# eloialonso/diamond

Hardware: AMD Instinct MI355X
Metric: imagined frames/sec (64x64, 3 denoise steps, batch 256) (higher is better)
Workload: dtype f32 via split-f16 MFMA (world-model convs (3x3 stride 1 / 2, 1x1): fp32 operands split into 2 x fp16 pieces, 3 x v_mfma_f32_*_f16 per product, fp32 accumulate (fp32-class, 22-bit operands); attention core, linears: exact fp32 v_mfma_f32_16x16x4_f32; actor-critic encoder forward, dgrad and weight-gra

## Files before the change

diamond_amd/csrc/dmd_common.h:

```cpp
#pragma once
#include <atomic>
#include <hip/hip_runtime.h>
#include <stdint.h>
#include <stdio.h>
#include <stdlib.h>

#include "../../include/diamond_hip.h"

typedef float f32x4 __attribute__((ext_vector_type(4)));

#define DMD_GN_EPS 1e-5
#define DMD_MAX_DEVICES 16

#ifndef DMD_DYNAMIC_LDS
#define DMD_DYNAMIC_LDS(type, name) extern __shared__ __attribute__((aligned(16))) type name[]
#endif

void dmd_set_error(const char* fmt, ...);

int dmd_env_generation();
struct DmdEnvInt {
  const char* name;
  int def;
  std::atomic<long long> gen_val{-1};
// ... 2 lines not shown
    long long gv = gen_val.load(std::memory_order_acquire);
    if (gv < 0 || (int)(gv >> 32) != g) {
      const char* e = getenv(name);
      const int v = e ? atoi(e) : def;
      gv = ((long long)g << 32) | (unsigned int)v;
      gen_val.store(gv, std::memory_order_release);
    }
    return (int)(unsigned int)(gv & 0xffffffffll);
  }
};

#define DMD_CHECK_ARG(cond, ...)  \
  do {                            \
    if (!(cond)) {                \
      dmd_set_error(__VA_ARGS__); \
      return 1;                   \
    }                             \
  } while (0)

#define DMD_LAUNCH_CHECK()                                            \
  do {                                                                \
    hipError_t e_ = hipGetLastError();                                \
    if (e_ != hipSuccess) {                                           \
      dmd_set_error("launch failed: %s", hipGetErrorString(e_));      \
      return 2;                                                       \
    }                                                                 \
  } while (0)

__device__ __forceinline__ float dmd_silu(float v) { return v / (1.0f + expf(-v)); }
__device__ __forceinline__ float dmd_silu_fast(float t) {
  return t * __builtin_amdgcn_rcpf(1.0f + __builtin_amdgcn_exp2f(-1.4426950408889634f * t));
}
__device__ __forceinline__ float dmd_sigmoid(float v) { return 1.0f / (1.0f + expf(-v)); }

__device__ __forceinline__ void dmd_finalize_stats(const double* st, int T, double count, float* mean, float* rstd) {
  double s = 0.0, ss = 0.0;
  for (int t = 0; t < T; ++t) {
    s += st[2 * t];
    ss += st[2 * t + 1];
  }
  const double m = s / count;
  double var = ss / count - m * m;
  var = var < 0.0 ? 0.0 : var;
  *mean = (float)m;
  *rstd = (float)(1.0 / sqrt(var + (double)DMD_GN_EPS));
}

__device__ __forceinline__ double dmd_wave_sum(double v) {
#pragma unroll
  for (int off = 32; off > 0; off >>= 1) v += __shfl_xor(v, off, 64);
  return v;
}

__host__ __device__ __forceinline__ int dmd_gn_groups(int C) { return C / DMD_GN_GROUP > 0 ? C / DMD_GN_GROUP : 1; }
__host__ __device__ __forceinline__ int dmd_gn_group_size(int C) { return C / dmd_gn_groups(C); }
__host__ __device__ __forceinline__ bool dmd_gn_width_ok(int C) {
  return C > 0 && C % 16 == 0 && C % dmd_gn_groups(C) == 0 && dmd_gn_group_size(C) % 4 == 0 && (C % DMD_GN_GROUP == 0 || C <= 256);
}

__device__ __forceinline__ void norm_entry_gs(const dmd_norm& nm, int n, int c, int C, int gs, double count, float* mean,
                                              float* a, float* add) {
  const int G = C / gs;
  const int g = c / gs;
  float m, rstd;
  dmd_finalize_stats(nm.stats + ((size_t)(n * G + g) * nm.stat_tiles) * 2, nm.stat_tiles, count, &m, &rstd);
  float mul = nm.mul ? nm.mul[(size_t)n * nm.mul_stride + c] : 1.0f;
// ... 19 lines not shown
```

diamond_amd/csrc/dmd_linear.hip:

```cpp
#include "dmd_common.h"

#define LIN_DEPTH 4
template <bool SPLITK>
__global__ __launch_bounds__(256) void linear_mfma_kernel(const dmd_linear_params p) {
  __shared__ f32x4 part[SPLITK ? 3 : 1][4][64];
  const int lane = threadIdx.x & 63, wave = threadIdx.x >> 6;
  const int i = lane & 15, kg = lane >> 4;
  const int m0 = SPLITK ? blockIdx.x * 32 : blockIdx.x * 64 + (wave >> 1) * 32;
  const int n0 = SPLITK ? blockIdx.y * 32 : blockIdx.y * 64 + (wave & 1) * 32;
  const int kq = SPLITK ? p.K >> 2 : p.K;
  const int kbase = SPLITK ? wave * kq : 0;
  const int nsteps = kq >> 4;
  f32x4 acc[2][2];
#pragma unroll
  for (int a = 0; a < 2; ++a)
#pragma unroll
    for (int b = 0; b < 2; ++b) acc[a][b] = (f32x4){0.f, 0.f, 0.f, 0.f};

  const float* arow[2];
  const float* wrow[2];
#pragma unroll
  for (int b = 0; b < 2; ++b) {
    int m = m0 + 16 * b + i;
    m = m < p.M ? m : p.M - 1;
    arow[b] = p.A + (size_t)m * p.lda + kbase + 4 * kg;
    int n = n0 + 16 * b + i;
    n = n < p.N ? n : p.N - 1;
    wrow[b] = p.W + (size_t)n * p.ldw + kbase + 4 * kg;
  }
  f32x4 af[LIN_DEPTH][2], wf[LIN_DEPTH][2];
#pragma unroll
  for (int d = 0; d < LIN_DEPTH; ++d) {
    const int ks = (d < nsteps ? d : nsteps - 1) * 16;
#pragma unroll
    for (int b = 0; b < 2; ++b) {
      af[d][b] = *(const f32x4*)(arow[b] + ks);
      wf[d][b] = *(const f32x4*)(wrow[b] + ks);
    }
  }
  for (int s0 = 0; s0 < nsteps; s0 += LIN_DEPTH) {
#pragma unroll
    for (int d = 0; d < LIN_DEPTH; ++d) {
// ... 32 lines not shown
        for (int mb = 0; mb < 2; ++mb) acc[nb][mb] += part[w][nb * 2 + mb][lane];
  }
#pragma unroll
  for (int nb = 0; nb < 2; ++nb)
#pragma unroll
    for (int mb = 0; mb < 2; ++mb) {
      const int m = m0 + 16 * mb + i;
      const int n = n0 + 16 * nb + 4 * kg;
      if (m >= p.M) continue;
#pragma unroll
      for (int r = 0; r < 4; ++r) {
        if (n + r >= p.N) continue;
        float v = acc[nb][mb][r];
        if (p.bias) v += p.bias[n + r];
        float* c = p.C + (size_t)m * p.ldc + n + r;
        if (p.accumulate) v += *c;
        if (p.silu) v = dmd_silu(v);
        *c = v;
      }
    }
}

extern "C" int dmd_linear(const dmd_linear_params* p, dmd_stream_t stream) {
  DMD_CHECK_ARG(p && p->A && p->W && p->C, "linear: null");
  DMD_CHECK_ARG(p->M > 0 && p->N > 0 && p->K > 0 && p->K % 16 == 0, "linear: bad M/N/K %d %d %d", p->M, p->N, p->K);
  DMD_CHECK_ARG(p->lda % 4 == 0 && p->ldw % 4 == 0, "linear: lda/ldw must be multiples of 4");
  if (p->K >= 512 && p->K % 64 == 0)
    hipLaunchKernelGGL(linear_mfma_kernel<true>, dim3((p->M + 31) / 32, (p->N + 31) / 32), dim3(256), 0, (hipStream_t)stream, *p);
  else
    hipLaunchKernelGGL(linear_mfma_kernel<false>, dim3((p->M + 63) / 64, (p->N + 63) / 64), dim3(256), 0, (hipStream_t)stream, *p);
  DMD_LAUNCH_CHECK();
  return 0;
}
```

diamond_amd/csrc/dmd_pointwise.hip:

```cpp
#include "dmd_common.h"

__global__ void edm_pack_input_kernel(const float* __restrict__ x, const float* __restrict__ obs,
                                      const float* __restrict__ cond, int cond_stride, float sd,
                                      float* __restrict__ out, int N, int Cx, int Cobs, int HW, int CPad, int T, int head) {
  const int Q = CPad >> 2, HW4 = HW >> 2;
  const size_t idx = (size_t)blockIdx.x * blockDim.x + threadIdx.x;
  if (idx >= (size_t)N * HW4 * Q) return;
  const int qd = idx % Q;
  const size_t npq = idx / Q;
  const int n = npq / HW4;
  const int pix0 = 4 * (int)(npq - (size_t)n * HW4);
  const float c_in = cond[(size_t)n * cond_stride + 0];
  const int cimg = Cobs / T;
  f32x4 t[4];
#pragma unroll
  for (int e = 0; e < 4; ++e) {
    const int cc = qd * 4 + e;
    t[e] = (f32x4){0.f, 0.f, 0.f, 0.f};
    if (cc < Cobs) {
      const int fr = cc / cimg, ci = cc - fr * cimg;
      int slot = fr + head;
      slot = slot >= T ? slot - T : slot;
      const f32x4 v = *(const f32x4*)(obs + ((size_t)n * Cobs + slot * cimg + ci) * HW + pix0);
#pragma unroll
// ... 215 lines not shown
  const int ox = op % Wo;
  const int oy = (op / Wo) % Ho;
  const int n = op / ((size_t)Wo * Ho);
  f32x4 best;
  int bi[4] = {0, 0, 0, 0};
#pragma unroll
  for (int k = 0; k < 4; ++k) {
    const int iy = oy * 2 + (k >> 1), ix = ox * 2 + (k & 1);
    const f32x4 v = *(const f32x4*)(x + (((size_t)n * H + iy) * W + ix) * C + cq * 4);
    if (k == 0)
      best = v;
    else {
#pragma unroll
      for (int e = 0; e < 4; ++e)
        if (v[e] > best[e] || v[e] != v[e]) {
          best[e] = v[e];
          bi[e] = k;
        }
    }
  }
  *(f32x4*)(out + op * C + cq * 4) = best;
  if (argmax) {
    uint32_t packed = bi[0] | (bi[1] << 8) | (bi[2] << 16) | (bi[3] << 24);
    *(uint32_t*)(argmax + op * C + cq * 4) = packed;
  }
}

__global__ void lstm_pointwise_kernel(const float* __restrict__ gates, const float* __restrict__ c_prev,
                                      float* __restrict__ h, float* __restrict__ c, int N, int Hd) {
  const int idx = blockIdx.x * blockDim.x + threadIdx.x;
  if (idx >= N * Hd) return;
  const int n = idx / Hd, k = idx - n * Hd;
  const float* gr = gates + (size_t)n * 4 * Hd;
  const float ig = dmd_sigmoid(gr[k]);
  const float fg = dmd_sigmoid(gr[Hd + k]);
  const float gg = tanhf(gr[2 * Hd + k]);
  const float og = dmd_sigmoid(gr[3 * Hd + k]);
  const float cn = fg * c_prev[idx] + ig * gg;
  c[idx] = cn;
  h[idx] = og * tanhf(cn);
}

__global__ void lstm_pointwise_bwd_kernel(const float* __restrict__ gates, const float* __restrict__ c_prev,
                                          const float* __restrict__ c_new, const float* __restrict__ dh,
                                          const float* __restrict__ dc, float* __restrict__ dgates, float* __restrict__ dc_prev,
                                          int N, int Hd) {
  const int idx = blockIdx.x * blockDim.x + threadIdx.x;
  if (idx >= N * Hd) return;
  const int n = idx / Hd, k = idx - n * Hd;
  const float* gr = gates + (size_t)n * 4 * Hd;
  const float ig = dmd_sigmoid(gr[k]);
  const float fg = dmd_sigmoid(gr[Hd + k]);
  const float gg = tanhf(gr[2 * Hd + k]);
  const float og = dmd_sigmoid(gr[3 * Hd + k]);
  const float tc = tanhf(c_new[idx]);
  const float dhv = dh ? dh[idx] : 0.f;
  const float dcv = (dc ? dc[idx] : 0.f) + dhv * og * (1.0f - tc * tc);
  float* dg = dgates + (size_t)n * 4 * Hd;
  dg[k] = dcv * gg * ig * (1.0f - ig);
  dg[Hd + k] = dcv * c_prev[idx] * fg * (1.0f - fg);
  dg[2 * Hd + k] = dcv * ig * (1.0f - gg * gg);
  dg[3 * Hd + k] = dhv * tc * og * (1.0f - og);
  dc_prev[idx] = dcv * fg;
}

__global__ void categorical_sample_kernel(const float* __restrict__ logits, const float* __restrict__ expo,
                                          int64_t* __restrict__ out, int N, int A) {
  const int n = blockIdx.x * blockDim.x + threadIdx.x;
  if (n >= N) return;
  const float* l = logits + (size_t)n * A;
  const float* e = expo + (size_t)n * A;
  float m = -INFINITY;
  for (int a = 0; a < A; ++a) m = fmaxf(m, l[a]);
// ... 386 lines not shown
```

diamond_amd/lstm_native.py:

```python
from __future__ import annotations

from typing import Optional, Tuple

import torch
import torch.nn.functional as F
from torch import Tensor

from . import engine as E
from . import native as nv


def _pad_k(t: Tensor) -> Tensor:
    k = t.shape[1]
    kp = (k + 15) // 16 * 16
    t = t.contiguous()
    return t if kp == k else F.pad(t, (0, kp - k))


def _mm_nt(a: Tensor, w: Tensor, bias: Optional[Tensor] = None, out: Optional[Tensor] = None, accumulate: bool = False) -> Tensor:
    a, w = _pad_k(a), _pad_k(w)
    return E.linear(a, w, bias, out=out, accumulate=accumulate)


class LstmHeadsFn(torch.autograd.Function):
    @staticmethod
    def forward(ctx, cache: E.PackCache, x: Tensor, hx: Tensor, cx: Tensor, w_ih: Tensor, w_hh: Tensor, b_ih: Tensor,
                b_hh: Tensor, w_heads: Tensor, b_heads: Tensor):
        x, hx, cx = x.detach().float().contiguous(), hx.detach().float().contiguous(), cx.detach().float().contiguous()
        n, hd = hx.shape
        gates = E.linear(x, w_ih.detach(), b_ih.detach())
        E.linear(hx, w_hh.detach(), b_hh.detach(), out=gates, accumulate=True)
        h = torch.empty_like(hx)
        c = torch.empty_like(cx)
        nv.check(nv.lib().dmd_lstm_pointwise(nv.fptr(gates), nv.fptr(cx), nv.fptr(h), nv.fptr(c), n, hd, nv.stream()),
                 "dmd_lstm_pointwise")
        heads = E.linear(h, w_heads.detach().contiguous(), b_heads.detach().contiguous())
        ctx.save_for_backward(x, hx, cx, gates, h, c, w_heads)
        ctx.w_ih_t = cache.get(w_ih, "T", lambda w: w.detach().t().contiguous()) if ctx.needs_input_grad[1] else None
        ctx.w_hh_t = cache.get(w_hh, "T", lambda w: w.detach().t().contiguous()) if ctx.needs_input_grad[2] else None
        return heads, h, c

    @staticmethod
    def backward(ctx, dheads: Optional[Tensor], dh: Optional[Tensor], dc: Optional[Tensor]):
        x, hx, cx, gates, h, c, w_heads = ctx.saved_tensors
        n, hd = hx.shape
        need = ctx.needs_input_grad
        dw_heads = db_heads = None
        dh_total = None if dh is None else dh.detach().float().contiguous()
        if dheads is not None:
            dheads = dheads.detach().float().contiguous()
            wt = w_heads.detach().t().contiguous()
            dh_total = _mm_nt(dheads, wt, out=dh_total.clone() if dh_total is not None else None, accumulate=dh_total is not None)
            dw_heads = _mm_nt(dheads.t(), h.t())
            db_heads = dheads.sum(0)
        dgates = torch.empty_like(gates)
        dc_prev = torch.empty_like(cx)
        dcc = None if dc is None else dc.detach().float().contiguous()
        nv.check(nv.lib().dmd_lstm_pointwise_bwd(nv.fptr(gates), nv.fptr(cx), nv.fptr(c), nv.fptr(dh_total), nv.fptr(dcc),
                                                 nv.fptr(dgates), nv.fptr(dc_prev), n, hd, nv.stream()), "dmd_lstm_pointwise_bwd")
        dx = dhx = None
        if need[1]:
            dx = _mm_nt(dgates, ctx.w_ih_t)
        if need[2]:
            dhx = _mm_nt(dgates, ctx.w_hh_t)
        dgt = dgates.t().contiguous()
        dw_ih = _mm_nt(dgt, x.t())
        dw_hh = _mm_nt(dgt, hx.t())
        db = dgates.sum(0)
        return (None, dx, dhx, dc_prev if need[3] else None, dw_ih, dw_hh, db, db, dw_heads, db_heads)


class LinearFn(torch.autograd.Function):

    @staticmethod
    def forward(ctx, cache: E.PackCache, x: Tensor, w: Tensor, b: Optional[Tensor]):
        x = x.detach().float().contiguous()
        y = _mm_nt(x, w.detach(), None if b is None else b.detach().contiguous())
        ctx.save_for_backward(x)
        ctx.w_t = (cache.get(w, "T", lambda t: t.detach().t().contiguous()) if isinstance(w, torch.nn.Parameter)
                   else w.detach().t().contiguous()) if ctx.needs_input_grad[1] else None
        ctx.has_bias = b is not None
        return y

    @staticmethod
    def backward(ctx, dy: Tensor):
        (x,) = ctx.saved_tensors
        dy = dy.detach().float().contiguous()
        dx = _mm_nt(dy, ctx.w_t) if ctx.needs_input_grad[1] else None
        dw = _mm_nt(dy.t(), x.t())
        return None, dx, dw, dy.sum(0) if ctx.has_bias else None


class LstmStepFn(torch.autograd.Function):

    @staticmethod
    def forward(ctx, cache: E.PackCache, gx: Tensor, hx: Tensor, cx: Tensor, w_hh: Tensor, b_hh: Tensor):
        hx, cx = hx.detach().float().contiguous(), cx.detach().float().contiguous()
        n, hd = hx.shape
        gates = gx.detach().float().clone(memory_format=torch.contiguous_format)
        E.linear(hx, w_hh.detach(), b_hh.detach(), out=gates, accumulate=True)
        h, c = torch.empty_like(hx), torch.empty_like(cx)
        nv.check(nv.lib().dmd_lstm_pointwise(nv.fptr(gates), nv.fptr(cx), nv.fptr(h), nv.fptr(c), n, hd, nv.stream()),
                 "dmd_lstm_pointwise")
        ctx.save_for_backward(hx, cx, gates, c)
        ctx.w_hh_t = cache.get(w_hh, "T", lambda w: w.detach().t().contiguous())
        return h, c

    @staticmethod
    def backward(ctx, dh: Optional[Tensor], dc: Optional[Tensor]):
        hx, cx, gates, c = ctx.saved_tensors
        n, hd = hx.shape
        dhc = None if dh is None else dh.detach().float().contiguous()
        dcc = None if dc is None else dc.detach().float().contiguous()
        dgates, dc_prev = torch.empty_like(gates), torch.empty_like(cx)
        nv.check(nv.lib().dmd_lstm_pointwise_bwd(nv.fptr(gates), nv.fptr(cx), nv.fptr(c), nv.fptr(dhc), nv.fptr(dcc),
                                                 nv.fptr(dgates), nv.fptr(dc_prev), n, hd, nv.stream()), "dmd_lstm_pointwise_bwd")
        need = ctx.needs_input_grad
        dhx = _mm_nt(dgates, ctx.w_hh_t) if need[2] else None
        dw_hh = _mm_nt(dgates.t(), hx.t())
        return None, dgates, dhx, dc_prev if need[3] else None, dw_hh, dgates.sum(0)


class LstmBurnInFn(torch.autograd.Function):

    @staticmethod
    def forward(ctx, cache: E.PackCache, x: Tensor, tb: int, w_ih: Tensor, w_hh: Tensor, b_ih: Tensor, b_hh: Tensor):
        x = x.detach().float().contiguous()
        k, hd = x.shape[0] // tb, w_hh.shape[1]
        gates = E.linear(x, w_ih.detach(), b_ih.detach())
        hs = torch.zeros(tb + 1, k, hd, device=x.device, dtype=torch.float32)
        cs = torch.zeros(tb + 1, k, hd, device=x.device, dtype=torch.float32)
        whh, bhh = w_hh.detach(), b_hh.detach()
        for i in range(tb):
            g = gates[i * k:(i + 1) * k]
            E.linear(hs[i], whh, bhh, out=g, accumulate=True)
            nv.check(nv.lib().dmd_lstm_pointwise(nv.fptr(g), nv.fptr(cs[i]), nv.fptr(hs[i + 1]), nv.fptr(cs[i + 1]), k, hd, nv.stream()),
                     "dmd_lstm_pointwise")
        ctx.save_for_backward(x, gates, hs, cs)
        ctx.tb = tb
        ctx.w_ih_t = cache.get(w_ih, "T", lambda w: w.detach().t().contiguous()) if ctx.needs_input_grad[1] else None
        ctx.w_hh_t = cache.get(w_hh, "T", lambda w: w.detach().t().contiguous())
        return hs[tb].clone(), cs[tb].clone()

    @staticmethod
    def backward(ctx, dh: Optional[Tensor], dc: Optional[Tensor]):
        x, gates, hs, cs = ctx.saved_tensors
        tb = ctx.tb
        k, hd = hs.shape[1], hs.shape[2]
        dgates = torch.empty_like(gates)
        dhc = torch.zeros(k, hd, device=x.device) if dh is None else dh.detach().float().contiguous()
        dcc = torch.zeros(k, hd, device=x.device) if dc is None else dc.detach().float().contiguous()
        for i in reversed(range(tb)):
            dg, dc_prev = dgates[i * k:(i + 1) * k], torch.empty_like(dcc)
            nv.check(nv.lib().dmd_lstm_pointwise_bwd(nv.fptr(gates[i * k:(i + 1) * k]), nv.fptr(cs[i]), nv.fptr(cs[i + 1]), nv.fptr(dhc), nv.fptr(dcc),
                                                     nv.fptr(dg), nv.fptr(dc_prev), k, hd, nv.stream()), "dmd_lstm_pointwise_bwd")
            dcc = dc_prev
            if i > 0:
                dhc = _mm_nt(dg, ctx.w_hh_t)
        dx = _mm_nt(dgates, ctx.w_ih_t) if ctx.needs_input_grad[1] else None
        dgt = dgates.t().contiguous()
        dw_ih = _mm_nt(dgt, x.t())
        dw_hh = _mm_nt(dgt[:, k:].contiguous(), hs[1:tb].reshape((tb - 1) * k, hd).t()) if tb > 1 else torch.zeros_like(ctx.w_hh_t.t())
        db = dgates.sum(0)
        return None, dx, None, dw_ih, dw_hh, db, db


def lstm_burn_in(cache: E.PackCache, x: Tensor, tb: int, lstm) -> Tuple[Tensor, Tensor]:
    nv.require_gpu(x)
    return LstmBurnInFn.apply(cache, x, tb, lstm.weight_ih, lstm.weight_hh, lstm.bias_ih, lstm.bias_hh)

# ... 42 lines not shown
```

diamond_amd/native.py:

```python
from __future__ import annotations

import ctypes as C
import os
from typing import Optional

import torch
from torch import Tensor

_HERE = os.path.dirname(os.path.abspath(__file__))
LIB_PATH = os.environ.get("DIAMOND_LIB", os.path.join(_HERE, "libdiamond_hip.so"))

PROLOGUE_NONE, PROLOGUE_NORM_SILU, PROLOGUE_NORM = 0, 1, 2
PRECISION_F32, PRECISION_F16X2 = 0, 1
GN_GROUP = 32


class NativeLibraryMissing(RuntimeError):
    pass


class Norm(C.Structure):
    _fields_ = [("stats", C.c_void_p), ("stat_tiles", C.c_int32), ("mul_plus_one", C.c_int32), ("mul", C.c_void_p),
                ("add", C.c_void_p), ("mul_stride", C.c_int64), ("add_stride", C.c_int64)]

# ... 52 lines not shown

CHECKSUM_PARTS = 8


class PoolRound(C.Structure):
    _fields_ = [("frames", C.c_void_p), ("pad", C.c_void_p), ("act", C.c_void_p), ("hx", C.c_void_p), ("cx", C.c_void_p),
                ("is_f32", C.c_int32), ("rows", C.c_int32)]


class ResetSlotsParams(C.Structure):
    _fields_ = [("B", C.c_int32), ("K", C.c_int32), ("T", C.c_int32), ("head", C.c_int32), ("per_frame", C.c_int64),
                ("hd", C.c_int32), ("reserved", C.c_int32), ("pool", PoolRound * 2), ("pool_base", C.c_int64), ("num_dead", C.c_void_p),
                ("slot_row", C.c_void_p), ("row_slot", C.c_void_p), ("next_obs", C.c_void_p), ("ctx", C.c_void_p),
                ("act_ring", C.c_void_p), ("hx", C.c_void_p), ("cx", C.c_void_p), ("enc_in", C.c_void_p)]


CHAIN_MAX_BLOCKS = 8


class ChainBlock(C.Structure):
    _fields_ = [("skip_slot", C.c_int32), ("save_slot", C.c_int32), ("film1_mul", C.c_int32 * 2), ("film1_add", C.c_int32 * 2),
                ("film2_mul", C.c_int32), ("film2_add", C.c_int32), ("has_attn", C.c_int32), ("reserved", C.c_int32),
                ("w1", C.c_void_p), ("w2", C.c_void_p), ("wproj", C.c_void_p), ("b1", C.c_void_p), ("b2", C.c_void_p),
                ("bproj", C.c_void_p), ("gn_gamma", C.c_void_p), ("gn_beta", C.c_void_p), ("wq", C.c_void_p), ("wk", C.c_void_p),
                ("wv", C.c_void_p), ("wo", C.c_void_p), ("bqkv", C.c_void_p), ("bo", C.c_void_p)]


class LowresChainParams(C.Structure):
    _fields_ = [("N", C.c_int32), ("nblocks", C.c_int32), ("input_save_slot", C.c_int32), ("reserved", C.c_int32),
                ("x", C.c_void_p), ("out", C.c_void_p), ("table", C.c_void_p), ("table_stride", C.c_int64),
                ("blocks", ChainBlock * CHAIN_MAX_BLOCKS)]


EXPORTS = (
    "dmd_conv2d", "dmd_conv2d_kernel_name", "dmd_conv2d_naive", "dmd_conv_stat_tiles", "dmd_pack_conv_weight", "dmd_conv2d_f16x2_eligible",
    "dmd_conv1x1_stream_eligible", "dmd_conv2d_proj_eligible", "dmd_pack_jobs", "dmd_checksums",
    "dmd_pack_conv_weight_f16x2", "dmd_linear", "dmd_attention", "dmd_attention_valid", "dmd_attention_bwd", "dmd_attention_bwd_valid",
    "dmd_attention_bwd_workspace_floats",
    "dmd_edm_pack_input", "dmd_cond_embed", "dmd_edm_denoised", "dmd_euler_step", "dmd_heun_step", "dmd_quantize_u8", "dmd_reset_state",
    "dmd_dequant_gather", "dmd_resolve_deaths", "dmd_reset_slots", "dmd_merge_slots", "dmd_merge_slots_bwd", "dmd_nchw_to_nhwc",
    "dmd_nhwc_to_nchw", "dmd_gn_stats", "dmd_gn_stats_valid", "dmd_maxpool2", "dmd_lstm_pointwise", "dmd_lstm_pointwise_bwd", "dmd_categorical_sample",
    "dmd_maxpool2_bwd", "dmd_gn_bwd_workspace_bytes", "dmd_gn_silu_bwd", "dmd_wgrad_workspace_floats", "dmd_conv2d_wgrad", "dmd_wgrad_job", "dmd_wgrad_reduce_jobs",
    "dmd_lowres_chain", "dmd_lowres_chain32", "dmd_last_error", "dmd_abi_version", "dmd_reload_env",
)

LAUNCHERS = frozenset(n for n in EXPORTS if n not in (
    "dmd_conv2d_kernel_name", "dmd_conv_stat_tiles", "dmd_conv2d_f16x2_eligible", "dmd_conv1x1_stream_eligible",
    "dmd_conv2d_proj_eligible", "dmd_attention_bwd_workspace_floats", "dmd_gn_bwd_workspace_bytes", "dmd_wgrad_workspace_floats", "dmd_wgrad_job", "dmd_last_error",
    "dmd_abi_version", "dmd_reload_env"))


class LaunchProfiler:

    def __init__(self) -> None:
        self.records = []
        self._pending = None

    def annotate(self, key: str, flops: float, nbytes: float) -> None:
        self._pending = (key, flops, nbytes)

    def call(self, name: str, fn, args):
        key, flops, nbytes = self._pending or (name, 0.0, 0.0)
        self._pending = None
        e0, e1 = torch.cuda.Event(enable_timing=True), torch.cuda.Event(enable_timing=True)
        e0.record()
        rc = fn(*args)
        e1.record()
        self.records.append((key, flops, nbytes, e0, e1))
        return rc

    def summary(self):
        torch.cuda.synchronize()
        out = {}
        for key, flops, nbytes, e0, e1 in self.records:
# ... 47 lines not shown
                                    C.c_int, C.c_void_p]
    L.dmd_attention_bwd_valid.argtypes = [C.c_void_p, C.c_void_p, C.c_void_p, C.c_void_p, C.c_void_p, C.c_int, C.c_int, C.c_int,
                                          C.c_int, C.c_int, C.c_int, C.c_int, C.c_void_p]
    L.dmd_attention_bwd_workspace_floats.argtypes = [C.c_int, C.c_int, C.c_int]
    L.dmd_attention_bwd_workspace_floats.restype = C.c_int64
    L.dmd_edm_pack_input.argtypes = [C.c_void_p, C.c_void_p, C.c_void_p, C.c_int, C.c_float, C.c_void_p, C.c_int, C.c_int,
                                     C.c_int, C.c_int, C.c_int, C.c_int, C.c_int, C.c_int, C.c_void_p]
    L.dmd_cond_embed.argtypes = [C.c_void_p, C.c_int, C.c_void_p, C.c_void_p, C.c_void_p, C.c_void_p, C.c_int,
                                 C.c_int, C.c_int, C.c_int, C.c_int, C.c_int, C.c_void_p]
    L.dmd_heun_step.argtypes = [C.c_void_p, C.c_void_p, C.c_void_p, C.c_void_p, C.c_float, C.c_float, C.c_float,
                                C.c_void_p, C.c_int64, C.c_void_p]
    L.dmd_quantize_u8.argtypes = [C.c_void_p, C.c_void_p, C.c_void_p, C.c_int64, C.c_void_p]
    L.dmd_dequant_gather.argtypes = [C.c_void_p, C.c_void_p, C.c_void_p, C.c_void_p, C.c_int, C.c_int, C.c_int64,
                                     C.c_int, C.c_void_p]
    L.dmd_reset_state.argtypes = [C.c_void_p, C.c_void_p, C.c_int, C.c_void_p, C.c_void_p, C.c_int, C.c_int, C.c_void_p, C.c_void_p,
                                  C.c_void_p, C.c_void_p, C.c_int, C.c_void_p, C.c_void_p]
    L.dmd_resolve_deaths.argtypes = [C.c_void_p, C.c_void_p, C.c_int, C.c_void_p, C.c_void_p, C.c_int, C.c_int, C.c_void_p, C.c_void_p,
                                     C.c_void_p, C.c_void_p]
    L.dmd_reset_slots.argtypes = [C.POINTER(ResetSlotsParams), C.c_void_p]
    L.dmd_merge_slots.argtypes = [C.c_void_p, C.c_void_p, C.c_void_p, C.c_void_p, C.c_int, C.c_int, C.c_void_p]
    L.dmd_merge_slots_bwd.argtypes = [C.c_void_p, C.c_void_p, C.c_void_p, C.c_void_p, C.c_void_p, C.c_int, C.c_int, C.c_int, C.c_void_p]
    L.dmd_edm_denoised.argtypes = [C.c_void_p, C.c_void_p, C.c_void_p, C.c_int, C.c_void_p, C.c_int, C.c_int64,
                                   C.c_void_p]
    L.dmd_euler_step.argtypes = [C.c_void_p, C.c_void_p, C.c_float, C.c_float, C.c_void_p, C.c_int64, C.c_void_p]
    L.dmd_nchw_to_nhwc.argtypes = [C.c_void_p, C.c_void_p, C.c_int, C.c_int, C.c_int, C.c_int, C.c_int, C.c_void_p]
    L.dmd_nhwc_to_nchw.argtypes = [C.c_void_p, C.c_void_p, C.c_int, C.c_int, C.c_int, C.c_int, C.c_int, C.c_void_p]
    L.dmd_gn_stats.argtypes = [C.c_void_p, C.c_void_p, C.c_int, C.c_int, C.c_int, C.c_void_p]
    L.dmd_gn_stats_valid.argtypes = [C.c_void_p, C.c_void_p, C.c_int, C.c_int, C.c_int, C.c_int, C.c_int, C.c_int, C.c_void_p]
    L.dmd_maxpool2.argtypes = [C.c_void_p, C.c_void_p, C.c_void_p, C.c_void_p, C.c_int, C.c_int, C.c_int, C.c_int,
                               C.c_void_p]
    L.dmd_lstm_pointwise.argtypes = [C.c_void_p, C.c_void_p, C.c_void_p, C.c_void_p, C.c_int, C.c_int, C.c_void_p]
    L.dmd_lstm_pointwise_bwd.argtypes = [C.c_void_p, C.c_void_p, C.c_void_p, C.c_void_p, C.c_void_p, C.c_void_p, C.c_void_p,
                                         C.c_int, C.c_int, C.c_void_p]
    L.dmd_categorical_sample.argtypes = [C.c_void_p, C.c_void_p, C.c_void_p, C.c_int, C.c_int, C.c_void_p]
    L.dmd_conv_stat_tiles.argtypes = [C.c_int, C.c_int]
    L.dmd_maxpool2_bwd.argtypes = [C.c_void_p, C.c_void_p, C.c_void_p, C.c_int, C.c_int, C.c_int, C.c_int, C.c_void_p]
    L.dmd_gn_bwd_workspace_bytes.argtypes = [C.c_int, C.c_int, C.c_int]
    L.dmd_gn_bwd_workspace_bytes.restype = C.c_int64
    L.dmd_gn_silu_bwd.argtypes = [C.POINTER(GnBwdParams), C.c_void_p]
    L.dmd_wgrad_workspace_floats.argtypes = [C.POINTER(WgradParams)]
    L.dmd_wgrad_workspace_floats.restype = C.c_int64
    L.dmd_conv2d_wgrad.argtypes = [C.POINTER(WgradParams), C.c_void_p]
    L.dmd_wgrad_job.argtypes = [C.POINTER(WgradParams), C.POINTER(WgradReduceJob)]
    L.dmd_wgrad_reduce_jobs.argtypes = [C.c_void_p, C.c_int, C.c_void_p]
    L.dmd_lowres_chain.argtypes = [C.POINTER(LowresChainParams), C.c_void_p]
    L.dmd_lowres_chain32.argtypes = [C.POINTER(LowresChainParams), C.c_void_p]


_lib: Optional[_Lib] = None


def lib() -> _Lib:
    global _lib
    if _lib is None:
        if not os.path.exists(LIB_PATH):
            raise NativeLibraryMissing(
                f"{LIB_PATH} not found: build it with `python -c 'import __graft_entry__ as g; g.build()'` "
                "(diamond_amd has no CPU/PyTorch fallback for its kernels)")
        L = C.CDLL(LIB_PATH)
        if hasattr(L, "dmd_simt_host_build"):
            raise NativeLibraryMissing(
                f"{LIB_PATH} is the SIMT-interpreter build of the kernels (tests/simt, test infrastructure): "
                "diamond_amd runs on libdiamond_hip.so only, there is no CPU path")
        declare_signatures(L)
        _lib = _Lib(L)
    return _lib
# ... 67 lines not shown
    cout, cin, k, _ = w_oihw.shape
    assert cout in (32, 64) and k in (1, 3), (cout, k)
    cinp = (cin + 15) // 16 * 16
    w = w_oihw.detach().contiguous().float()
    out = torch.empty(cinp // 16 * k * k * 2 * cout * 16, device=w.device, dtype=torch.float16)
    check(lib().dmd_pack_conv_weight_f16x2(fptr(w), ptr(out), cout, cin, k, cinp, stream()), "dmd_pack_conv_weight_f16x2")
    return out


def pad_vector(v: Optional[Tensor], n: int) -> Optional[Tensor]:
    if v is None:
        return None
    out = torch.zeros(n, device=v.device, dtype=torch.float32)
    out[: v.numel()] = v.detach().float()
    return out


def linear(a: Tensor, w: Tensor, bias: Optional[Tensor], out: Tensor, accumulate: bool = False, silu: bool = False) -> Tensor:
    p = LinearParams()
    p.M, p.K = a.shape
    p.N = w.shape[0]
    assert w.shape[1] == p.K and out.shape == (p.M, p.N), (a.shape, w.shape, out.shape)
    assert a.stride(1) == 1 and w.stride(1) == 1 and out.stride(1) == 1
    p.A, p.lda = ptr(a), a.stride(0)
    p.W, p.ldw = ptr(w), w.stride(0)
    p.bias = ptr(bias)
    p.C, p.ldc = ptr(out), out.stride(0)
    p.accumulate, p.silu = int(accumulate), int(silu)
    if PROFILER is not None:
        PROFILER.annotate(f"linear_mfma_kernel<{'true' if p.K >= 512 else 'false'}>", 2.0 * p.M * p.N * p.K,
                          4.0 * (p.M * p.K + p.N * p.K + p.M * p.N))
    check(lib().dmd_linear(C.byref(p), stream()), "dmd_linear")
    return out
```

diamond_amd/rew_end_model.py:

```python
from __future__ import annotations

from dataclasses import dataclass
from typing import List, Optional, Tuple

import torch
from torch import Tensor, nn

from . import engine as E
from . import native as nv
from .blocks import Downsample, FilmTable, ResBlocks, RunCtx, conv3x3


@dataclass
class RewEndModelConfig:
    lstm_dim: int
    img_channels: int
    img_size: int
    cond_channels: int
    depths: List[int]
    channels: List[int]
    attn_depths: List[int]
    num_actions: Optional[int] = None


# ... 114 lines not shown

    @torch.no_grad()
    def predict_rew_end(self, obs: Tensor, act: Tensor, next_obs: Tensor,
                        hx_cx: Optional[Tuple[Tensor, Tensor]] = None) -> Tuple[Tensor, Tensor, Tuple[Tensor, Tensor]]:
        b, t, c, h, w = obs.shape
        dev = obs.device
        nv.check_current_device(dev)
        x = torch.cat((obs.reshape(b * t, c, h, w), next_obs.reshape(b * t, c, h, w)), dim=1)
        nd = len(self.encoder.downsamples) - 2
        hp, wp = E.padded_extent(h, w, nd)
        valid = None if (hp, wp) == (h, w) else (h, w)
        if valid is not None:
            assert h % 2 ** nd == 0 and w % 2 ** nd == 0, f"RewEndModel: {h}x{w} is not a multiple of {2 ** nd} (the reference's own constraint)"
            x = torch.nn.functional.pad(x, (0, wp - w, 0, hp - h))
        x16 = E.nchw_to_nhwc(x, 16)
        cond = self._cache.f32(self.act_emb.weight)[act.reshape(b * t)].contiguous()
        if self._film is None:
            self._film = FilmTable(self.encoder)
        ctx = RunCtx(self._cache, self._film, self._film.compute(cond))
        fa = self.encoder.run(ctx, x16, valid)
        ft = fa.t if fa.valid is None else fa.t[:, :fa.valid[0], :fa.valid[1]].contiguous()
        feat = ft.reshape(b, t, -1)
        hd = self.cfg.lstm_dim
        if hx_cx is None:
            hx = torch.zeros(b, hd, device=dev)
            cx = torch.zeros(b, hd, device=dev)
        else:
            hx, cx = hx_cx[0][0].contiguous(), hx_cx[1][0].contiguous()
        w_ih, w_hh = self._lstm_in_weight(), self._cache.f32(self.lstm.weight_hh_l0)
        b_ih, b_hh = self._cache.f32(self.lstm.bias_ih_l0), self._cache.f32(self.lstm.bias_hh_l0)
        gates_x = E.linear(feat.reshape(b * t, -1), w_ih, b_ih).reshape(b, t, 4 * hd)
        ys = []
        for i in range(t):
            g = gates_x[:, i].contiguous()
            E.linear(hx, w_hh, b_hh, out=g, accumulate=True)
            hn, cn = torch.empty_like(hx), torch.empty_like(cx)
            nv.check(nv.lib().dmd_lstm_pointwise(nv.fptr(g), nv.fptr(cx), nv.fptr(hn), nv.fptr(cn), b, hd, nv.stream()),
                     "dmd_lstm_pointwise")
            hx, cx = hn, cn
            ys.append(hx)
        y = torch.stack(ys, dim=1).reshape(b * t, hd)
        y = E.linear(y, self._cache.f32(self.head[0].weight), self._cache.f32(self.head[0].bias), silu=True)
        logits = E.linear(y, self._cache.f32(self.head[2].weight), None).reshape(b, t, -1)
        return logits[:, :, :-2], logits[:, :, -2:], (hx.unsqueeze(0), cx.unsqueeze(0))

    def logits_with_grad(self, obs: Tensor, act: Tensor, next_obs: Tensor, precision: Optional[str] = None) -> Tensor:
        import torch.nn.functional as F
        from . import unet_train as UT
        from .blocks import AdaGroupNorm
        from .lstm_native import LinearFn, LstmStepFn

        b, t, c, h, w = obs.shape
        x = torch.cat((obs.reshape(b * t, c, h, w), next_obs.reshape(b * t, c, h, w)), dim=1).detach()
        nd = len(self.encoder.downsamples) - 2
        hp, wp = E.padded_extent(h, w, nd)
        valid = None if (hp, wp) == (h, w) else (h, w)
        if valid is not None:
            assert h % 2 ** nd == 0 and w % 2 ** nd == 0, f"RewEndModel: {h}x{w} is not a multiple of {2 ** nd} (the reference's own constraint)"
            x = F.pad(x, (0, wp - w, 0, hp - h))
        x16 = E.nchw_to_nhwc(x, 16)
        cond = self.act_emb(act.reshape(b * t))
        if self._film is None:
            self._film = FilmTable(self.encoder)
        film = self._film
        table = LinearFn.apply(self._cache, cond, torch.cat([m.linear.weight for m in film.norms], dim=0),
                               torch.cat([m.linear.bias for m in film.norms], dim=0))
        if self._train_params is None:
            skip = {id(p) for m in self.encoder.modules() if isinstance(m, AdaGroupNorm) for p in m.parameters()}
            self._train_params = [p for p in self.encoder.parameters() if id(p) not in skip]
        precision = precision or UT.TRAIN_PRECISION

# ... 58 lines not shown
```

include/diamond_hip.h:

```cpp
#ifndef DIAMOND_HIP_H
#define DIAMOND_HIP_H

#include <stdint.h>

#ifdef __cplusplus
extern "C" {
#endif

typedef void* dmd_stream_t;

#define DMD_PROLOGUE_NONE 0
#define DMD_PROLOGUE_NORM_SILU 1
#define DMD_PROLOGUE_NORM 2

#define DMD_GN_GROUP 32

typedef struct dmd_norm {
  const double* stats;
  int32_t stat_tiles;
  int32_t mul_plus_one;
  const float* mul;
  const float* add;
  int64_t mul_stride;
  int64_t add_stride;
// ... 161 lines not shown
  int32_t B, K, T, head;
  int64_t per_frame;
  int32_t hd, reserved;
  dmd_pool_round pool[2];
  int64_t pool_base;
  const int32_t* num_dead;
  const int64_t* slot_row;
  const int32_t* row_slot;
  const float* next_obs;
  float* ctx;
  int64_t* act_ring;
  float* hx;
  float* cx;
  float* enc_in;
} dmd_reset_slots_params;
int dmd_reset_slots(const dmd_reset_slots_params* p, dmd_stream_t stream);

int dmd_merge_slots(const float* base, const float* slots, const int32_t* row_slot, float* out, int B, int D, dmd_stream_t stream);
int dmd_merge_slots_bwd(const float* d_out, const int32_t* row_slot, const int64_t* slot_row, float* d_base, float* d_slots, int B, int K,
                        int D, dmd_stream_t stream);

int dmd_nchw_to_nhwc(const float* in, float* out, int N, int C, int H, int W, int CPad, dmd_stream_t stream);
int dmd_nhwc_to_nchw(const float* in, float* out, int N, int C, int H, int W, int CPad, dmd_stream_t stream);

int dmd_gn_stats(const float* x, double* stats, int N, int HW, int C, dmd_stream_t stream);
int dmd_gn_stats_valid(const float* x, double* stats, int N, int H, int W, int valid_h, int valid_w, int C, dmd_stream_t stream);

int dmd_maxpool2(const float* x, float* out, uint8_t* argmax, double* out_stats, int N, int H, int W, int C,
                 dmd_stream_t stream);

int dmd_lstm_pointwise(const float* gates, const float* c_prev, float* h, float* c, int N, int Hd,
                       dmd_stream_t stream);

int dmd_lstm_pointwise_bwd(const float* gates, const float* c_prev, const float* c_new, const float* dh, const float* dc,
                           float* dgates, float* dc_prev, int N, int Hd, dmd_stream_t stream);

int dmd_categorical_sample(const float* logits, const float* expo, int64_t* out, int N, int A, dmd_stream_t stream);


int dmd_maxpool2_bwd(const float* dpooled, const uint8_t* argmax, float* dx, int N, int H, int W, int C,
                     dmd_stream_t stream);

typedef struct dmd_gn_bwd_params {
  int32_t N, HW, C;
  int32_t identity_activation;
  const float* x;
  dmd_norm norm;
  const float* da;
  const float* dskip;
  float* dx;
  void* workspace;
  float* dmul;
  float* dadd;
  int32_t W, valid_h, valid_w, reserved;
} dmd_gn_bwd_params;
int64_t dmd_gn_bwd_workspace_bytes(int N, int HW, int C);
int dmd_gn_silu_bwd(const dmd_gn_bwd_params* p, dmd_stream_t stream);

typedef struct dmd_wgrad_params {
  int32_t N, H, W;
  int32_t Cout;
  int32_t taps;
  int32_t cin_real;
  dmd_conv_src src;
  const float* dy;
  float* workspace;
// ... 28 lines not shown
```

Baseline: 13000.

## Fuse LSTM gate GEMMs, bias and pointwise update into one cell kernel

Adds an lstm_cell kernel that computes the input and hidden gate GEMMs with fp32 MFMA, split-K across waves for large K, adds the biases, writes the gates and applies the LSTM nonlinearity in one launch. It replaces the separate linear, accumulate-linear and pointwise launches (plus a gates clone or contiguous copy) in the actor-critic and reward/end LSTM paths. It also adds an XCD-aware workgroup ordering helper, used by the new kernel and available to the linear kernel only behind a compile flag. The aim is fewer launches and fewer round trips of the gate tensor per timestep, at the cost of a larger per-block tile covering four gates with possibly lower occupancy.

Measured after the change: 12680. -2.5%, worse.

```diff
diff --git a/diamond_amd/csrc/dmd_common.h b/diamond_amd/csrc/dmd_common.h
--- a/diamond_amd/csrc/dmd_common.h
+++ b/diamond_amd/csrc/dmd_common.h
@@ -58,6 +58,19 @@
   return t * __builtin_amdgcn_rcpf(1.0f + __builtin_amdgcn_exp2f(-1.4426950408889634f * t));
 }
 __device__ __forceinline__ float dmd_sigmoid(float v) { return 1.0f / (1.0f + expf(-v)); }
+__device__ __forceinline__ void dmd_lstm_unit(float gi, float gf, float gg_, float go, float c_prev, float* h, float* c) {
+  const float ig = dmd_sigmoid(gi);
+  const float fg = dmd_sigmoid(gf);
+  const float gg = tanhf(gg_);
+  const float og = dmd_sigmoid(go);
+  const float cn = fg * c_prev + ig * gg;
+  *c = cn;
+  *h = og * tanhf(cn);
+}
+__device__ __forceinline__ int dmd_xcd_order(int hw, int nwg) {
+  const int q = nwg >> 3, r = nwg & 7, x = hw & 7;
+  return (x < r ? x * (q + 1) : r * (q + 1) + (x - r) * q) + (hw >> 3);
+}
 
 __device__ __forceinline__ void dmd_finalize_stats(const double* st, int T, double count, float* mean, float* rstd) {
   double s = 0.0, ss = 0.0;
diff --git a/diamond_amd/csrc/dmd_linear.hip b/diamond_amd/csrc/dmd_linear.hip
--- a/diamond_amd/csrc/dmd_linear.hip
+++ b/diamond_amd/csrc/dmd_linear.hip
@@ -6,8 +6,14 @@
   __shared__ f32x4 part[SPLITK ? 3 : 1][4][64];
   const int lane = threadIdx.x & 63, wave = threadIdx.x >> 6;
   const int i = lane & 15, kg = lane >> 4;
-  const int m0 = SPLITK ? blockIdx.x * 32 : blockIdx.x * 64 + (wave >> 1) * 32;
-  const int n0 = SPLITK ? blockIdx.y * 32 : blockIdx.y * 64 + (wave & 1) * 32;
+#ifdef DMD_LINEAR_XCD_ORDER
+  const int id = dmd_xcd_order(blockIdx.x + blockIdx.y * gridDim.x, gridDim.x * gridDim.y);
+  const int bx = id % gridDim.x, by = id / gridDim.x;
+#else
+  const int bx = blockIdx.x, by = blockIdx.y;
+#endif
+  const int m0 = SPLITK ? bx * 32 : bx * 64 + (wave >> 1) * 32;
+  const int n0 = SPLITK ? by * 32 : by * 64 + (wave & 1) * 32;
   const int kq = SPLITK ? p.K >> 2 : p.K;
   const int kbase = SPLITK ? wave * kq : 0;
   const int nsteps = kq >> 4;
@@ -106,3 +112,141 @@
   DMD_LAUNCH_CHECK();
   return 0;
 }
+
+__device__ __forceinline__ bool cell_gemm(f32x4 (&acc)[4][2], const float* A, int64_t lda, const float* W, int64_t ldw, int K, int M,
+                                          int Hd, int m0, int u0, int wave, int i, int kg) {
+  const bool split = K >= 512 && K % 64 == 0;
+  const int kq = split ? K >> 2 : K;
+  const int kbase = split ? wave * kq : 0;
+  const int nsteps = (split || wave == 0) ? kq >> 4 : 0;
+  if (nsteps == 0) return split;
+  const float* arow[2];
+  const float* wrow[4];
+#pragma unroll
+  for (int b = 0; b < 2; ++b) {
+    int m = m0 + 16 * b + i;
+    m = m < M ? m : M - 1;
+    arow[b] = A + (size_t)m * lda + kbase + 4 * kg;
+  }
+#pragma unroll
+  for (int g = 0; g < 4; ++g) wrow[g] = W + (size_t)(g * Hd + u0 + i) * ldw + kbase + 4 * kg;
+  f32x4 af[LIN_DEPTH][2], wf[LIN_DEPTH][4];
+#pragma unroll
+  for (int d = 0; d < LIN_DEPTH; ++d) {
+    const int ks = (d < nsteps ? d : nsteps - 1) * 16;
+#pragma unroll
+    for (int b = 0; b < 2; ++b) af[d][b] = *(const f32x4*)(arow[b] + ks);
+#pragma unroll
+    for (int g = 0; g < 4; ++g) wf[d][g] = *(const f32x4*)(wrow[g] + ks);
+  }
+  for (int s0 = 0; s0 < nsteps; s0 += LIN_DEPTH) {
+#pragma unroll
+    for (int d = 0; d < LIN_DEPTH; ++d) {
+      if (s0 + d < nsteps) {
+#pragma unroll
+        for (int g = 0; g < 4; ++g)
+#pragma unroll
+          for (int mb = 0; mb < 2; ++mb)
+#pragma unroll
+            for (int t = 0; t < 4; ++t)
+              acc[g][mb] = __builtin_amdgcn_mfma_f32_16x16x4f32(wf[d][g][t], af[d][mb][t], acc[g][mb], 0, 0, 0);
+        const int sn = s0 + d + LIN_DEPTH;
+        const int ks = (sn < nsteps ? sn : nsteps - 1) * 16;
+#pragma unroll
+        for (int b = 0; b < 2; ++b) af[d][b] = *(const f32x4*)(arow[b] + ks);
+#pragma unroll
+        for (int g = 0; g < 4; ++g) wf[d][g] = *(const f32x4*)(wrow[g] + ks);
+      }
+    }
+  }
+  return split;
+}
+
+__global__ __launch_bounds__(256) void lstm_cell_kernel(const dmd_lstm_cell_params p) {
+  __shared__ f32x4 part[3][16][64];
+  const int lane = threadIdx.x & 63, wave = threadIdx.x >> 6;
+  const int i = lane & 15, kg = lane >> 4;
+  const int mblocks = (p.M + 31) / 32;
+  const int id = dmd_xcd_order(blockIdx.x, gridDim.x);
+  const int m0 = (id % mblocks) * 32, u0 = (id / mblocks) * 16;
+  f32x4 ax[4][2], ah[4][2];
+#pragma unroll
+  for (int g = 0; g < 4; ++g)
+#pragma unroll
+    for (int b = 0; b < 2; ++b) ax[g][b] = ah[g][b] = (f32x4){0.f, 0.f, 0.f, 0.f};
+  const bool split_x = p.x ? cell_gemm(ax, p.x, p.ldx, p.w_ih, p.ldw_ih, p.Kx, p.M, p.Hd, m0, u0, wave, i, kg) : false;
+  const bool split_h = cell_gemm(ah, p.hx, p.ldh, p.w_hh, p.ldw_hh, p.Hd, p.M, p.Hd, m0, u0, wave, i, kg);
+  if (wave) {
+#pragma unroll
+    for (int g = 0; g < 4; ++g)
+#pragma unroll
+      for (int b = 0; b < 2; ++b) {
+        if (split_x) part[wave - 1][g * 2 + b][lane] = ax[g][b];
+        if (split_h) part[wave - 1][8 + g * 2 + b][lane] = ah[g][b];
+      }
+  }
+  __syncthreads();
+  if (wave) return;
+#pragma unroll
+  for (int w = 0; w < 3; ++w)
+#pragma unroll
+    for (int g = 0; g < 4; ++g)
+#pragma unroll
+      for (int b = 0; b < 2; ++b) {
+        if (split_x) ax[g][b] += part[w][g * 2 + b][lane];
+        if (split_h) ah[g][b] += part[w][8 + g * 2 + b][lane];
+      }
+  const int u = u0 + 4 * kg;
+#pragma unroll
+  for (int mb = 0; mb < 2; ++mb) {
+    const int m = m0 + 16 * mb + i;
+    if (m >= p.M) continue;
+    f32x4 pre[4];
+#pragma unroll
+    for (int g = 0; g < 4; ++g) {
+      const int n = g * p.Hd + u;
+      const f32x4 vx = p.x ? ax[g][mb] : *(const f32x4*)(p.gx + (size_t)m * p.ldgx + n);
+#pragma unroll
+      for (int r = 0; r < 4; ++r) {
+        float a = vx[r];
+        if (p.x && p.b_ih) a += p.b_ih[n + r];
+        float v = ah[g][mb][r];
+        if (p.b_hh) v += p.b_hh[n + r];
+        pre[g][r] = v + a;
+      }
+      *(f32x4*)(p.gates + (size_t)m * p.ldg + n) = pre[g];
+    }
+    const size_t o = (size_t)m * p.Hd + u;
+    const f32x4 cp = *(const f32x4*)(p.c_prev + o);
+    f32x4 hn, cn;
+#pragma unroll
+    for (int r = 0; r < 4; ++r) {
+      float hv, cv;
+      dmd_lstm_unit(pre[0][r], pre[1][r], pre[2][r], pre[3][r], cp[r], &hv, &cv);
+      hn[r] = hv;
+      cn[r] = cv;
+    }
+    *(f32x4*)(p.h + o) = hn;
+    *(f32x4*)(p.c + o) = cn;
+  }
+}
+
+static inline bool aligned16(const void* q) { return ((uintptr_t)q & 15) == 0; }
+
+extern "C" int dmd_lstm_cell(const dmd_lstm_cell_params* p, dmd_stream_t stream) {
+  DMD_CHECK_ARG(p && p->hx && p->w_hh && p->c_prev && p->gates && p->h && p->c, "lstm_cell: null");
+  DMD_CHECK_ARG(p->M > 0 && p->Hd > 0 && p->Hd % 16 == 0, "lstm_cell: bad M/Hd %d %d", p->M, p->Hd);
+  if (p->x) {
+    DMD_CHECK_ARG(p->w_ih && p->Kx > 0 && p->Kx % 16 == 0, "lstm_cell: bad Kx %d", p->Kx);
+    DMD_CHECK_ARG(p->ldx % 4 == 0 && p->ldw_ih % 4 == 0 && aligned16(p->x) && aligned16(p->w_ih), "lstm_cell: x / w_ih rows must be 16-byte aligned");
+  } else {
+    DMD_CHECK_ARG(p->gx && p->ldgx % 4 == 0 && aligned16(p->gx), "lstm_cell: neither x nor an aligned gx");
+  }
+  DMD_CHECK_ARG(p->ldh % 4 == 0 && p->ldw_hh % 4 == 0 && p->ldg % 4 == 0, "lstm_cell: ldh/ldw_hh/ldg must be multiples of 4");
+  DMD_CHECK_ARG(aligned16(p->hx) && aligned16(p->w_hh) && aligned16(p->c_prev) && aligned16(p->gates) && aligned16(p->h) && aligned16(p->c),
+                "lstm_cell: pointers must be 16-byte aligned");
+  const int nwg = ((p->M + 31) / 32) * (p->Hd / 16);
+  hipLaunchKernelGGL(lstm_cell_kernel, dim3(nwg), dim3(256), 0, (hipStream_t)stream, *p);
+  DMD_LAUNCH_CHECK();
+  return 0;
+}
diff --git a/diamond_amd/csrc/dmd_pointwise.hip b/diamond_amd/csrc/dmd_pointwise.hip
--- a/diamond_amd/csrc/dmd_pointwise.hip
+++ b/diamond_amd/csrc/dmd_pointwise.hip
@@ -271,13 +271,7 @@
   if (idx >= N * Hd) return;
   const int n = idx / Hd, k = idx - n * Hd;
   const float* gr = gates + (size_t)n * 4 * Hd;
-  const float ig = dmd_sigmoid(gr[k]);
-  const float fg = dmd_sigmoid(gr[Hd + k]);
-  const float gg = tanhf(gr[2 * Hd + k]);
-  const float og = dmd_sigmoid(gr[3 * Hd + k]);
-  const float cn = fg * c_prev[idx] + ig * gg;
-  c[idx] = cn;
-  h[idx] = og * tanhf(cn);
+  dmd_lstm_unit(gr[k], gr[Hd + k], gr[2 * Hd + k], gr[3 * Hd + k], c_prev[idx], h + idx, c + idx);
 }
 
 __global__ void lstm_pointwise_bwd_kernel(const float* __restrict__ gates, const float* __restrict__ c_prev,
diff --git a/diamond_amd/lstm_native.py b/diamond_amd/lstm_native.py
--- a/diamond_amd/lstm_native.py
+++ b/diamond_amd/lstm_native.py
@@ -28,12 +28,10 @@
                 b_hh: Tensor, w_heads: Tensor, b_heads: Tensor):
         x, hx, cx = x.detach().float().contiguous(), hx.detach().float().contiguous(), cx.detach().float().contiguous()
         n, hd = hx.shape
-        gates = E.linear(x, w_ih.detach(), b_ih.detach())
-        E.linear(hx, w_hh.detach(), b_hh.detach(), out=gates, accumulate=True)
+        gates = torch.empty(n, 4 * hd, device=x.device, dtype=torch.float32)
         h = torch.empty_like(hx)
         c = torch.empty_like(cx)
-        nv.check(nv.lib().dmd_lstm_pointwise(nv.fptr(gates), nv.fptr(cx), nv.fptr(h), nv.fptr(c), n, hd, nv.stream()),
-                 "dmd_lstm_pointwise")
+        nv.lstm_cell(x, w_ih.detach(), b_ih.detach(), None, hx, w_hh.detach(), b_hh.detach(), cx, gates, h, c)
         heads = E.linear(h, w_heads.detach().contiguous(), b_heads.detach().contiguous())
         ctx.save_for_backward(x, hx, cx, gates, h, c, w_heads)
         ctx.w_ih_t = cache.get(w_ih, "T", lambda w: w.detach().t().contiguous()) if ctx.needs_input_grad[1] else None
@@ -97,11 +95,12 @@
     def forward(ctx, cache: E.PackCache, gx: Tensor, hx: Tensor, cx: Tensor, w_hh: Tensor, b_hh: Tensor):
         hx, cx = hx.detach().float().contiguous(), cx.detach().float().contiguous()
         n, hd = hx.shape
-        gates = gx.detach().float().clone(memory_format=torch.contiguous_format)
-        E.linear(hx, w_hh.detach(), b_hh.detach(), out=gates, accumulate=True)
+        gx = gx.detach().float()
+        if gx.stride(1) != 1 or gx.stride(0) % 4 or gx.data_ptr() % 16:
+            gx = gx.contiguous()
+        gates = torch.empty(n, 4 * hd, device=hx.device, dtype=torch.float32)
         h, c = torch.empty_like(hx), torch.empty_like(cx)
-        nv.check(nv.lib().dmd_lstm_pointwise(nv.fptr(gates), nv.fptr(cx), nv.fptr(h), nv.fptr(c), n, hd, nv.stream()),
-                 "dmd_lstm_pointwise")
+        nv.lstm_cell(None, None, None, gx, hx, w_hh.detach(), b_hh.detach(), cx, gates, h, c)
         ctx.save_for_backward(hx, cx, gates, c)
         ctx.w_hh_t = cache.get(w_hh, "T", lambda w: w.detach().t().contiguous())
         return h, c
@@ -133,9 +132,7 @@
         whh, bhh = w_hh.detach(), b_hh.detach()
         for i in range(tb):
             g = gates[i * k:(i + 1) * k]
-            E.linear(hs[i], whh, bhh, out=g, accumulate=True)
-            nv.check(nv.lib().dmd_lstm_pointwise(nv.fptr(g), nv.fptr(cs[i]), nv.fptr(hs[i + 1]), nv.fptr(cs[i + 1]), k, hd, nv.stream()),
-                     "dmd_lstm_pointwise")
+            nv.lstm_cell(None, None, None, g, hs[i], whh, bhh, cs[i], g, hs[i + 1], cs[i + 1])
         ctx.save_for_backward(x, gates, hs, cs)
         ctx.tb = tb
         ctx.w_ih_t = cache.get(w_ih, "T", lambda w: w.detach().t().contiguous()) if ctx.needs_input_grad[1] else None
diff --git a/diamond_amd/native.py b/diamond_amd/native.py
--- a/diamond_amd/native.py
+++ b/diamond_amd/native.py
@@ -108,6 +108,14 @@
                 ("blocks", ChainBlock * CHAIN_MAX_BLOCKS)]
 
 
+class LstmCellParams(C.Structure):
+    _fields_ = [("M", C.c_int32), ("Hd", C.c_int32), ("Kx", C.c_int32), ("reserved", C.c_int32),
+                ("x", C.c_void_p), ("ldx", C.c_int64), ("w_ih", C.c_void_p), ("ldw_ih", C.c_int64), ("b_ih", C.c_void_p),
+                ("gx", C.c_void_p), ("ldgx", C.c_int64), ("hx", C.c_void_p), ("ldh", C.c_int64),
+                ("w_hh", C.c_void_p), ("ldw_hh", C.c_int64), ("b_hh", C.c_void_p), ("c_prev", C.c_void_p),
+                ("gates", C.c_void_p), ("ldg", C.c_int64), ("h", C.c_void_p), ("c", C.c_void_p)]
+
+
 EXPORTS = (
     "dmd_conv2d", "dmd_conv2d_kernel_name", "dmd_conv2d_naive", "dmd_conv_stat_tiles", "dmd_pack_conv_weight", "dmd_conv2d_f16x2_eligible",
     "dmd_conv1x1_stream_eligible", "dmd_conv2d_proj_eligible", "dmd_pack_jobs", "dmd_checksums",
@@ -115,7 +123,7 @@
     "dmd_attention_bwd_workspace_floats",
     "dmd_edm_pack_input", "dmd_cond_embed", "dmd_edm_denoised", "dmd_euler_step", "dmd_heun_step", "dmd_quantize_u8", "dmd_reset_state",
     "dmd_dequant_gather", "dmd_resolve_deaths", "dmd_reset_slots", "dmd_merge_slots", "dmd_merge_slots_bwd", "dmd_nchw_to_nhwc",
-    "dmd_nhwc_to_nchw", "dmd_gn_stats", "dmd_gn_stats_valid", "dmd_maxpool2", "dmd_lstm_pointwise", "dmd_lstm_pointwise_bwd", "dmd_categorical_sample",
+    "dmd_nhwc_to_nchw", "dmd_gn_stats", "dmd_gn_stats_valid", "dmd_maxpool2", "dmd_lstm_pointwise", "dmd_lstm_pointwise_bwd", "dmd_lstm_cell", "dmd_categorical_sample",
     "dmd_maxpool2_bwd", "dmd_gn_bwd_workspace_bytes", "dmd_gn_silu_bwd", "dmd_wgrad_workspace_floats", "dmd_conv2d_wgrad", "dmd_wgrad_job", "dmd_wgrad_reduce_jobs",
     "dmd_lowres_chain", "dmd_lowres_chain32", "dmd_last_error", "dmd_abi_version", "dmd_reload_env",
 )
@@ -229,6 +237,7 @@
     L.dmd_lstm_pointwise.argtypes = [C.c_void_p, C.c_void_p, C.c_void_p, C.c_void_p, C.c_int, C.c_int, C.c_void_p]
     L.dmd_lstm_pointwise_bwd.argtypes = [C.c_void_p, C.c_void_p, C.c_void_p, C.c_void_p, C.c_void_p, C.c_void_p, C.c_void_p,
                                          C.c_int, C.c_int, C.c_void_p]
+    L.dmd_lstm_cell.argtypes = [C.POINTER(LstmCellParams), C.c_void_p]
     L.dmd_categorical_sample.argtypes = [C.c_void_p, C.c_void_p, C.c_void_p, C.c_int, C.c_int, C.c_void_p]
     L.dmd_conv_stat_tiles.argtypes = [C.c_int, C.c_int]
     L.dmd_maxpool2_bwd.argtypes = [C.c_void_p, C.c_void_p, C.c_void_p, C.c_int, C.c_int, C.c_int, C.c_int, C.c_void_p]
@@ -362,3 +371,26 @@
                           4.0 * (p.M * p.K + p.N * p.K + p.M * p.N))
     check(lib().dmd_linear(C.byref(p), stream()), "dmd_linear")
     return out
+
+
+def lstm_cell(x: Optional[Tensor], w_ih: Optional[Tensor], b_ih: Optional[Tensor], gx: Optional[Tensor], hx: Tensor, w_hh: Tensor,
+              b_hh: Optional[Tensor], c_prev: Tensor, gates: Tensor, h: Tensor, c: Tensor) -> None:
+    p = LstmCellParams()
+    p.M, p.Hd = hx.shape
+    assert w_hh.shape == (4 * p.Hd, p.Hd) and gates.shape == (p.M, 4 * p.Hd), (hx.shape, w_hh.shape, gates.shape)
+    assert hx.stride(1) == 1 and w_hh.stride(1) == 1 and gates.stride(1) == 1
+    if x is not None:
+        p.Kx = x.shape[1]
+        assert x.shape[0] == p.M and w_ih.shape == (4 * p.Hd, p.Kx) and x.stride(1) == 1 and w_ih.stride(1) == 1, (x.shape, w_ih.shape)
+        p.x, p.ldx, p.w_ih, p.ldw_ih, p.b_ih = ptr(x), x.stride(0), ptr(w_ih), w_ih.stride(0), fptr(b_ih)
+    else:
+        assert gx.shape == gates.shape and gx.stride(1) == 1, (gx.shape, gx.stride())
+        p.gx, p.ldgx = ptr(gx), gx.stride(0)
+    p.hx, p.ldh, p.w_hh, p.ldw_hh, p.b_hh = ptr(hx), hx.stride(0), ptr(w_hh), w_hh.stride(0), fptr(b_hh)
+    p.c_prev, p.gates, p.ldg, p.h, p.c = fptr(c_prev), ptr(gates), gates.stride(0), fptr(h), fptr(c)
+    for t in (x, w_ih, gx, hx, w_hh, gates):
+        assert t is None or t.dtype == torch.float32, t.dtype
+    if PROFILER is not None:
+        k = p.Kx + p.Hd
+        PROFILER.annotate("lstm_cell_kernel", 2.0 * p.M * 4 * p.Hd * k, 4.0 * (p.M * k + 4 * p.Hd * k + p.M * 6 * p.Hd))
+    check(lib().dmd_lstm_cell(C.byref(p), stream()), "dmd_lstm_cell")
diff --git a/diamond_amd/rew_end_model.py b/diamond_amd/rew_end_model.py
--- a/diamond_amd/rew_end_model.py
+++ b/diamond_amd/rew_end_model.py
@@ -170,11 +170,9 @@
         gates_x = E.linear(feat.reshape(b * t, -1), w_ih, b_ih).reshape(b, t, 4 * hd)
         ys = []
         for i in range(t):
-            g = gates_x[:, i].contiguous()
-            E.linear(hx, w_hh, b_hh, out=g, accumulate=True)
+            g = gates_x[:, i]
             hn, cn = torch.empty_like(hx), torch.empty_like(cx)
-            nv.check(nv.lib().dmd_lstm_pointwise(nv.fptr(g), nv.fptr(cx), nv.fptr(hn), nv.fptr(cn), b, hd, nv.stream()),
-                     "dmd_lstm_pointwise")
+            nv.lstm_cell(None, None, None, g, hx, w_hh, b_hh, cx, g, hn, cn)
             hx, cx = hn, cn
             ys.append(hx)
         y = torch.stack(ys, dim=1).reshape(b * t, hd)
diff --git a/include/diamond_hip.h b/include/diamond_hip.h
--- a/include/diamond_hip.h
+++ b/include/diamond_hip.h
@@ -217,6 +217,22 @@
 int dmd_lstm_pointwise(const float* gates, const float* c_prev, float* h, float* c, int N, int Hd,
                        dmd_stream_t stream);
 
+typedef struct dmd_lstm_cell_params {
+  int32_t M, Hd, Kx;
+  int32_t reserved;
+  const float* x; int64_t ldx;
+  const float* w_ih; int64_t ldw_ih;
+  const float* b_ih;
+  const float* gx; int64_t ldgx;
+  const float* hx; int64_t ldh;
+  const float* w_hh; int64_t ldw_hh;
+  const float* b_hh;
+  const float* c_prev;
+  float* gates; int64_t ldg;
+  float* h; float* c;
+} dmd_lstm_cell_params;
+int dmd_lstm_cell(const dmd_lstm_cell_params* p, dmd_stream_t stream);
+
 int dmd_lstm_pointwise_bwd(const float* gates, const float* c_prev, const float* c_new, const float* dh, const float* dc,
                            float* dgates, float* dc_prev, int N, int Hd, dmd_stream_t stream);
 
```
